# PacificBiosciences/portello

Hardware: AMD Instinct MI355X
Metric: lifted HiFi reads/sec (whole node) (higher is better)
Workload: dtype int32; 1 GPU; wgs30x; reads_total=2000000, reads_this_rank=2000000, read_len_mean=15000, items_per_gpu=2065417, in_ops_per_gpu=62827345, out_ops_per_gpu=56590310, large_items_per_gpu=0, mid_items_per_gpu=0, retry_items_per_gpu=0, lane_items_per_gpu=2065417, heavy_lane_items_per_gpu=0, seq_fmt=bam4, parallelism=one read set, 20 Mb windows dealt to 1 ranks by input ops, gather=none, launched_by=single process

## Files before the change

include/portello_liftover.h:

```cpp
#ifndef PORTELLO_LIFTOVER_H
#define PORTELLO_LIFTOVER_H

#include <stddef.h>
#include <stdint.h>

#ifdef __cplusplus
extern "C" {
#endif

#define PLO_API_VERSION 20

typedef enum plo_status {
    PLO_OK = 0,
    PLO_ERR_INVALID_ARG = 1,
    PLO_ERR_NO_DEVICE = 2,
    PLO_ERR_HIP = 3,
    PLO_ERR_OUT_OF_MEMORY = 4,
    PLO_ERR_RANGE = 5,
    PLO_ERR_INTERNAL = 6,
    PLO_ERR_IO = 7,
    PLO_ERR_DATA = 8
} plo_status;

enum {
    PLO_ITEM_LIFTED = 0,
    PLO_ITEM_NO_LIFTOVER = 1,
    PLO_ITEM_LEN_MISMATCH = 2,
    PLO_ITEM_PANIC = 3,
    PLO_ITEM_NEED_BASES = 4
};

enum {
    PLO_SEQ_BAM4 = 0,
// ... 92 lines not shown
    uint32_t n_big_items;
    uint64_t n_in_ops;
    uint64_t n_out_ops;
    uint64_t algo_bytes;
    float lanes_ms;
    float retry_ms;
    uint32_t n_lane_items;
    uint32_t n_retry_items;
    float mid_ms;
    uint32_t n_mid_items;
    uint32_t n_miss_items;
    float miss_ms;
    uint32_t tile_cap;
    uint32_t tile_window;
    float heavy_lanes_ms;
    uint32_t n_heavy_lane_items;
    float lane_utilisation;
    uint32_t heavy_kernel;
    uint32_t host_syncs;
} plo_timing;

plo_status plo_index_create(const plo_index_desc *desc, int device, plo_index **out);
void plo_index_destroy(plo_index *index);
plo_status plo_index_segment_map(const plo_index *index, uint32_t global_seg, uint32_t cap, int64_t *keys,
                                 int64_t *vals, uint32_t *n_entries);

plo_status plo_ctx_create(const plo_index *index, void *hip_stream, plo_ctx **out);
void plo_ctx_destroy(plo_ctx *ctx);
plo_status plo_ctx_set_stats(plo_ctx *ctx, int on);
plo_status plo_ctx_set_phase_events(plo_ctx *ctx, int on);

plo_status plo_liftover_batch(plo_ctx *ctx, const plo_batch_in *in, uint32_t stages, plo_batch_out *out);
plo_status plo_liftover_batch_dev(plo_ctx *ctx, const plo_batch_in *in, uint32_t stages, plo_batch_out *out);

typedef struct plo_finish_in {
    const uint16_t *read_flags;
    const uint8_t *qual;
    const uint64_t *read_qual_off;
    uint64_t qual_bytes;
} plo_finish_in;

#define PLO_NO_FLIP UINT64_MAX

typedef struct plo_finish_out {
    const uint16_t *item_flag;
    const uint16_t *item_bin;
// ... 509 lines not shown
```

portello_amd/abi.py:

```python
from __future__ import annotations

import ctypes as C
from dataclasses import dataclass, field
from typing import List, Optional, Sequence

import numpy as np

PLO_OK = 0
PLO_ERR_INVALID_ARG = 1
PLO_ERR_NO_DEVICE = 2
PLO_ERR_HIP = 3
PLO_ERR_OUT_OF_MEMORY = 4
PLO_ERR_RANGE = 5
PLO_ERR_INTERNAL = 6
PLO_ERR_IO = 7
PLO_ERR_DATA = 8

ITEM_LIFTED = 0
ITEM_NO_LIFTOVER = 1
ITEM_LEN_MISMATCH = 2
ITEM_PANIC = 3
ITEM_NEED_BASES = 4

SEQ_BAM4 = 0
# ... 85 lines not shown
        ("item_cseg", _u32p),
        ("seq_full", _u8p),
        ("read_seq_full_off", _u64p),
    ]


class PloBatchOut(C.Structure):
    _fields_ = [
        ("n_items", C.c_uint32),
        ("item_seg", _u32p),
        ("item_cseg", _u32p),
        ("item_status", _u8p),
        ("item_need_flipped", _u8p),
        ("item_mapq", _u8p),
        ("item_chrom_index", _u32p),
        ("item_ref_pos", _i64p),
        ("item_cigar_off", _u64p),
        ("item_cigar_len", _u32p),
        ("cigar", _u32p),
        ("n_cigar", C.c_uint64),
    ]


PLO_API_VERSION = 20


class PloTiming(C.Structure):
    _fields_ = [
        ("struct_size", C.c_uint32),
        ("total_ms", C.c_float),
        ("enumerate_ms", C.c_float),
        ("lift_ms", C.c_float),
        ("big_ms", C.c_float),
        ("n_items", C.c_uint32),
        ("n_big_items", C.c_uint32),
        ("n_in_ops", C.c_uint64),
        ("n_out_ops", C.c_uint64),
        ("algo_bytes", C.c_uint64),
        ("lanes_ms", C.c_float),
        ("retry_ms", C.c_float),
        ("n_lane_items", C.c_uint32),
        ("n_retry_items", C.c_uint32),
        ("mid_ms", C.c_float),
        ("n_mid_items", C.c_uint32),
        ("n_miss_items", C.c_uint32),
        ("miss_ms", C.c_float),
        ("tile_cap", C.c_uint32),
# ... 516 lines not shown
```

portello_amd/api.py:

```python
from __future__ import annotations

import ctypes as C
import os
from typing import Callable, List, Optional, Sequence, Tuple

import numpy as np

from . import abi
from . import cigar as cg

_HERE = os.path.dirname(os.path.abspath(__file__))
LIB_PATH = os.environ.get("PLO_LIB") or os.path.join(_HERE, "libportello_liftover.so")

Backend = Callable[[abi.IndexData, abi.BatchData, int], abi.BatchResult]


class PortelloError(RuntimeError):
    def __init__(self, status: int, msg: str):
        super().__init__(f"portello_liftover status {status}: {msg}")
        self.status = status


_lib = None


def load_library(path: Optional[str] = None):
    global _lib
    if _lib is not None and path is None:
        return _lib
    path = path or LIB_PATH
    if not os.path.exists(path):
        raise PortelloError(abi.PLO_ERR_NO_DEVICE, f"{path} not built: run `python -m portello_amd.build` (hipcc, gfx950)")
    try:
        import torch
    except ImportError:
        pass
    L = C.CDLL(path)
    vp = C.c_void_p
    if not hasattr(L, "plo_api_version") or L.plo_api_version() != abi.PLO_API_VERSION:
        raise PortelloError(abi.PLO_ERR_INVALID_ARG, f"{path} was built for another PLO_API_VERSION than this binding ({abi.PLO_API_VERSION}): rebuild it")
    L.plo_index_create.restype = C.c_int
    L.plo_index_create.argtypes = [C.POINTER(abi.PloIndexDesc), C.c_int, C.POINTER(vp)]
    L.plo_index_destroy.restype = None
    L.plo_index_destroy.argtypes = [vp]
    L.plo_index_segment_map.restype = C.c_int
    L.plo_index_segment_map.argtypes = [vp, C.c_uint32, C.c_uint32, C.POINTER(C.c_int64), C.POINTER(C.c_int64), C.POINTER(C.c_uint32)]
    L.plo_ctx_create.restype = C.c_int
    L.plo_ctx_create.argtypes = [vp, vp, C.POINTER(vp)]
    L.plo_ctx_destroy.restype = None
    L.plo_ctx_destroy.argtypes = [vp]
    L.plo_liftover_batch.restype = C.c_int
    L.plo_liftover_batch.argtypes = [vp, C.POINTER(abi.PloBatchIn), C.c_uint32, C.POINTER(abi.PloBatchOut)]
    L.plo_liftover_batch_dev.restype = C.c_int
    L.plo_liftover_batch_dev.argtypes = [vp, C.POINTER(abi.PloBatchIn), C.c_uint32, C.POINTER(abi.PloBatchOut)]
    L.plo_compact_output_dev.restype = C.c_int
    L.plo_compact_output_dev.argtypes = [vp, C.POINTER(abi.PloBatchOut)]
    L.plo_host_alloc.restype = C.c_int
    L.plo_host_alloc.argtypes = [C.c_size_t, C.POINTER(C.c_void_p)]
    L.plo_host_free.restype = None
    L.plo_host_free.argtypes = [C.c_void_p]
    L.plo_sa_segments_dev.restype = C.c_int
    L.plo_sa_segments_dev.argtypes = [vp, C.POINTER(abi.PloSaIn), C.POINTER(abi.PloSaOut)]
    L.plo_finish_batch_dev.restype = C.c_int
    L.plo_finish_batch_dev.argtypes = [vp, C.POINTER(abi.PloBatchIn), C.POINTER(abi.PloFinishIn), C.POINTER(abi.PloFinishOut)]
    L.plo_nm_dev.restype = C.c_int
    L.plo_nm_dev.argtypes = [vp, C.POINTER(abi.PloBatchIn), C.POINTER(abi.PloNmOut)]
    L.plo_md_dev.restype = C.c_int
# ... 93 lines not shown

    def __init__(self, data: abi.IndexData, device: int = 0):
        self.lib = load_library()
        self.data = data
        self._desc = data.to_desc()
        h = C.c_void_p()
        st = self.lib.plo_index_create(C.byref(self._desc), device, C.byref(h))
        if st != abi.PLO_OK:
            raise PortelloError(st, "plo_index_create failed" + (" (no usable HIP device)" if st == abi.PLO_ERR_NO_DEVICE else ""))
        self.handle = h
        self.device = device

    def segment_map(self, global_seg: int) -> Tuple[np.ndarray, np.ndarray]:
        n = C.c_uint32(0)
        self.lib.plo_index_segment_map(self.handle, global_seg, 0, None, None, C.byref(n))
        keys = np.zeros(max(1, n.value), dtype=np.int64)
        vals = np.zeros(max(1, n.value), dtype=np.int64)
        st = self.lib.plo_index_segment_map(self.handle, global_seg, n.value, keys.ctypes.data_as(C.POINTER(C.c_int64)),
                                            vals.ctypes.data_as(C.POINTER(C.c_int64)), C.byref(n))
        if st != abi.PLO_OK:
            raise PortelloError(st, "plo_index_segment_map")
        return keys[: n.value], vals[: n.value]

    def close(self):
        if getattr(self, "handle", None):
            self.lib.plo_index_destroy(self.handle)
            self.handle = None

    def __del__(self):
        try:
            self.close()
        except Exception:
            pass


class Engine:

    def __init__(self, index: Index, stream: Optional[int] = None):
        self.lib = index.lib
        self.index = index
        h = C.c_void_p()
        st = self.lib.plo_ctx_create(index.handle, C.c_void_p(stream) if stream else None, C.byref(h))
        if st != abi.PLO_OK:
            raise PortelloError(st, "plo_ctx_create failed")
        self.handle = h

# ... 373 lines not shown
```

portello_amd/build.py:

```python
from __future__ import annotations

import os
import subprocess
import sys

HERE = os.path.dirname(os.path.abspath(__file__))
CSRC = os.path.join(HERE, "csrc")
LIB = os.path.join(HERE, "libportello_liftover.so")
SOURCES = ["engine.hip", "bam_host.cpp", "phase1.cpp", "gather_rccl.cpp"]
LIBS = ["-lz", "-ldl"]
HEADERS = ["plo_wave.hpp", "lift_core.hpp", "lane_core.hpp", "lane_stream.hpp", "inflate.hpp", "deflate.hpp", "finish_core.hpp", "records_core.hpp", "batch_core.hpp", "aln_walk.hpp", "nm_core.hpp", "md_core.hpp", "eqx_core.hpp", "sort_core.hpp", "merge_core.hpp", "index_core.hpp", "depth_core.hpp", "pileup_core.hpp", "fasta_core.hpp", "window_core.hpp", "bgzf_walk.hpp", "lift_types.hpp", "index_pack.hpp", "enumerate.hpp", "bam_internal.hpp"]


def hipcc() -> str:
    for cand in (os.environ.get("HIPCC"), "/opt/rocm/bin/hipcc", "hipcc"):
        if cand and (os.path.isabs(cand) and os.path.exists(cand) or not os.path.isabs(cand)):
            return cand
    return "hipcc"


def source_hash() -> str:
    import hashlib

    h = hashlib.sha256()
    for f in sorted(["engine.hip"] + [x for x in HEADERS if x != "bam_internal.hpp"]):
        with open(os.path.join(CSRC, f), "rb") as fh:
            h.update(f.encode() + b"\0" + fh.read())
    return h.hexdigest()[:16]


def build_timing() -> str:
    out = os.path.join(HERE, "libportello_liftover_timing.so")
    cmd = [hipcc(), "--offload-arch=gfx950", "-O3", "-std=c++17", "-fPIC", "-shared", "-DPLO_PHASE_TIMING", "-I" + CSRC, "-o", out,
           os.path.join(CSRC, "engine.hip"), os.path.join(CSRC, "bam_host.cpp"), os.path.join(CSRC, "phase1.cpp"), os.path.join(CSRC, "gather_rccl.cpp")] + LIBS
# ... 21 lines not shown
```

portello_amd/csrc/engine.hip:

```cpp
#include <hip/hip_runtime.h>

#include <plo_wave.hpp>
#include <stdio.h>
#include <string.h>

#include <algorithm>
#include <atomic>
#include <chrono>
#include <map>
#include <mutex>
#include <string>
#include <vector>

#include "enumerate.hpp"
#include "finish_core.hpp"
#include "records_core.hpp"
#include "batch_core.hpp"
#include "nm_core.hpp"
#include "md_core.hpp"
#include "eqx_core.hpp"
#include "sort_core.hpp"
#include "merge_core.hpp"
#include "index_core.hpp"
#include "depth_core.hpp"
// ... 117 lines not shown
    if (bad) n = 0;
    seg_reflen[s] = (int)part;
    seg_readlen[s] = rpart > 0xfffffffeull ? 0xffffffffu : (uint32_t)rpart;
    seg_nm[s] = (c1 - c0) - pairs;
    seg_cnt[s] = n;
}

__global__ void k_item_emit(DevIndex ix, DevBatch bt, DevWork wk, uint32_t stages, const uint32_t *seg_off, int *seg_reflen, uint32_t item_cap, uint32_t *err) {
    uint32_t s = blockIdx.x * blockDim.x + threadIdx.x;
    if (s >= bt.n_segs) return;
    const uint32_t o0 = seg_off[s], o1 = seg_off[s + 1];
    if (o1 > item_cap) {
        if (o1 > o0) atomicOr(err, (uint32_t)VERR_CAP);
        return;
    }
    const int ref_len = seg_reflen[s];
    SegInfo si;
    seg_info_level0(si, bt, wk, stages, s);
    if (o0 == o1) return;
    seg_info_level1(si, ix, bt, wk, stages, s);
    bool neg = false;
    emit_segment_items(ix, wk, stages, s, o0, (long long)ref_len, si, &neg);
    if (neg) atomicOr(err, (uint32_t)VERR_RANGE);
}

__global__ __launch_bounds__(64) void k_map_build(const uint32_t *seg_cigar, const uint32_t *seg_cigar_off, const int64_t *seg_pos, uint32_t n_segments,
                                                  const uint32_t *kv_off, KV *kv, int *counts) {
    for (uint32_t g = blockIdx.x; g < n_segments; g += gridDim.x) {
        const uint32_t c0 = seg_cigar_off[g], c1 = seg_cigar_off[g + 1];
        const int cnt = build_segment_map_wave(seg_cigar + c0, c1 - c0, (long long)seg_pos[g], kv ? kv + kv_off[g] : nullptr);
        if (counts && threadIdx.x == 0) counts[g] = cnt;
    }
}

__global__ void k_item_desc(DevIndex ix, DevBatch bt, DevWork wk, uint32_t stages, const uint32_t *in_seg, const uint32_t *in_cseg,
                            uint32_t *err) {
    uint32_t i = blockIdx.x * blockDim.x + threadIdx.x;
    if (i >= wk.n_items) return;
    uint32_t seg = in_seg[i];
    {
        bool ok = seg < bt.n_segs;
        if (ok) {
            uint32_t contig = bt.seg_contig[seg];
            ok = contig < ix.n_contigs && in_cseg[i] < ix.contig_seg_off[contig + 1] - ix.contig_seg_off[contig];
        }
        if (!ok) {
// ... 1282 lines not shown

struct AlnPass {
    DevBuf len, off, partial;
    DevBuf out;
    DevBuf blk;
    HostBuf h;
    hipEvent_t ev[4] = {nullptr, nullptr, nullptr, nullptr};
    void release() {
        for (DevBuf *b : {&len, &off, &partial, &out, &blk}) b->release();
        h.release();
        for (hipEvent_t e : ev)
            if (e) (void)hipEventDestroy(e);
    }
};

}

struct plo_index {
    int device = 0;
    PackedIndex host;
    DevIndex d{};
    std::vector<void *> owned;
    uint32_t max_segs_per_contig = 0;
};

struct plo_fasta {
    int device = 0;
    hipStream_t stream = nullptr;
    hipEvent_t ev[6] = {nullptr, nullptr, nullptr, nullptr, nullptr, nullptr};
    bool emit_timed = false;
    bool byte_stores = false;
    std::string err;
    FaHost h;
    DevBuf text, tile_fn, tile_state, cnt, start, partial, blk, hdr, dest;
    HostBuf h_blk, h_hdr, h_dest;
    uint8_t *out = nullptr;
    size_t out_cap = 0;
    float ms = 0.f;
    bool finished = false;
    std::vector<int64_t> o_len;
    std::vector<const uint8_t *> o_ptr;
    std::vector<void *> adopted;
};

struct plo_depth {
    int device = 0;
// ... 355 lines not shown
            ix->owned.push_back(p);
            if (desc->chrom_len[c] > 0 && hipMemcpy(p, src, (size_t)desc->chrom_len[c], hipMemcpyHostToDevice) != hipSuccess)
                return fail(PLO_ERR_HIP);
            chrom_ptr[c] = (const uint8_t *)p;
        }
    }
    for (uint32_t c = 0; c < desc->n_contigs; ++c) {
        const uint8_t *src = desc->rev_contig_seq ? desc->rev_contig_seq[c] : nullptr;
        if (!src) continue;
        if (desc->seq_mem == PLO_MEM_DEVICE) {
            rev_ptr[c] = src;
        } else {
            void *p = nullptr;
            size_t bytes = std::max<size_t>((size_t)desc->contig_len[c], 16);
            if (hipMalloc(&p, bytes) != hipSuccess) return fail(PLO_ERR_OUT_OF_MEMORY);
            ix->owned.push_back(p);
            if (desc->contig_len[c] > 0 && hipMemcpy(p, src, (size_t)desc->contig_len[c], hipMemcpyHostToDevice) != hipSuccess)
                return fail(PLO_ERR_HIP);
            rev_ptr[c] = (const uint8_t *)p;
        }
    }
    if (upload(ix->owned, chrom_ptr, &d.chrom_seq) != hipSuccess) return fail(PLO_ERR_HIP);
    if (upload(ix->owned, rev_ptr, &d.contig_revseq) != hipSuccess) return fail(PLO_ERR_HIP);
    *out = ix;
    return PLO_OK;
}

void plo_index_destroy(plo_index *ix) {
    if (!ix) return;
    (void)hipSetDevice(ix->device);
    for (void *p : ix->owned) (void)hipFree(p);
    delete ix;
}

static thread_local std::string g_fasta_err;
#define FA_TRY(f, call)                                                                 \
    do {                                                                                \
        hipError_t _e = (call);                                                         \
        if (_e != hipSuccess) {                                                         \
            (f)->err = std::string(#call) + ": " + hipGetErrorString(_e);               \
            return (_e == hipErrorOutOfMemory) ? PLO_ERR_OUT_OF_MEMORY : PLO_ERR_HIP;   \
        }                                                                               \
    } while (0)

static void fasta_release(plo_fasta *f) {
    (void)hipSetDevice(f->device);
    if (f->stream) (void)hipStreamSynchronize(f->stream);
    for (DevBuf *b : {&f->text, &f->tile_fn, &f->tile_state, &f->cnt, &f->start, &f->partial, &f->blk, &f->hdr, &f->dest}) b->release();
    for (HostBuf *b : {&f->h_blk, &f->h_hdr, &f->h_dest}) b->release();
// ... 3529 lines not shown
```

portello_amd/csrc/lane_core.hpp:

```cpp
#pragma once
#include <plo_wave.hpp>
#include <stdint.h>

#include <type_traits>
#ifdef PLO_EMULATOR
#include <stdio.h>
#include <stdlib.h>
#endif

#include "lift_core.hpp"

#ifdef PLO_EMULATOR
#define PLO_MARK(s)
#else
#define PLO_MARK(s) asm volatile("; " s)
#endif

#ifndef PLO_SHIFT_LOCKSTEP
#define PLO_SHIFT_LOCKSTEP 1
#endif

namespace plo {



#ifdef PLO_EMULATOR
struct __attribute__((packed, aligned(4))) Ops4 {
    uint32_t x, y, z, w;
};
#else
typedef uint32_t Ops4 __attribute__((ext_vector_type(4), aligned(4)));
#endif
struct LaneOut {
// ... 127 lines not shown
            const bool keep = act & (t != OP_D);
            t = (t == OP_I) ? (int)OP_S : t;
            const bool same = keep & (run >= 16u) & (t == (int)(run & 15u));
            const bool flush = keep & !same & (run >= 16u);
            if (flush) o.R[w] = run;
            w += flush ? 1 : 0;
            const uint32_t add = (t == OP_P) ? 0u : ((uint32_t)L << 4);
            run = same ? run + add : (keep ? mk_op(t, L) : run);
        }
        {
            const bool flush = fix & (run >= 16u);
            if (flush) o.R[w] = run;
            w += flush ? 1 : 0;
            o.no = fix ? w : o.no;
        }
    }
}

struct XW16 {
    Ops4 r4, q4;
    uint32_t r1, q1;
    int rsh, qsh, jmin;
};
PLO_DEV bool xw16_issue(bool on, const uint8_t *ref, int ref_len, int r0, const ReadSeq &rd, int q0, const uint8_t *safe, XW16 &w, bool &miss) {
    bool ok = on & (r0 >= 0) & (q0 >= 0) & (q0 <= rd.len - 16);
    const int rsh = (int)(((unsigned)(uintptr_t)ref + (unsigned)r0) & 3u);
    ok = ok & (r0 - rsh >= 0) & (r0 - rsh <= ref_len - 20);
    const int jmin = rd.flip ? rd.len - q0 - 16 : q0;
    const bool bam4 = rd.fmt != PLO_SEQ_ASCII;
    int b0 = bam4 ? (jmin >> 1) : jmin;
    miss = false;
    if (rd.fmt == PLO_SEQ_BAM4_SPARSE) {
        const int j0 = ok ? jmin : 0, j1 = ok ? jmin + 15 : 0;
        const int g0 = j0 >> 5, g1 = j1 >> 5;
        const PLO_GLOBAL uint32_t *hdr = (const PLO_GLOBAL uint32_t *)(ok ? rd.p : safe);
        const uint32_t m0 = hdr[2 * (g0 >> 5)], rk0 = hdr[2 * (g0 >> 5) + 1], m1 = hdr[2 * (g1 >> 5)];
        const bool present = (((m0 >> (g0 & 31)) & (m1 >> (g1 & 31))) & 1u) != 0u;
        const unsigned rank = rk0 + (unsigned)__builtin_popcount(m0 & ((1u << (g0 & 31)) - 1u));
        const long long off = (long long)rd.data + (long long)rank * 16 + ((j0 >> 1) & 15);
        const bool bad = !present | (rank > 0x3ffffffu) | (off + (g1 - g0) * 16 + 20 > (long long)rd.hi);
        miss = ok & bad;
        ok = ok & !bad;
        b0 = (int)off;
    }
    const int qsh = (int)(((unsigned)(uintptr_t)rd.p + (unsigned)b0) & 3u);
    ok = ok & (b0 - qsh >= rd.lo) & (b0 - qsh + 20 <= rd.hi);
#ifdef PLO_EXP_PROBE_NOMEM
    const PLO_GLOBAL uint32_t *pr = (const PLO_GLOBAL uint32_t *)safe;
    const PLO_GLOBAL uint32_t *pq = (const PLO_GLOBAL uint32_t *)safe;
#else
    const PLO_GLOBAL uint32_t *pr = (const PLO_GLOBAL uint32_t *)(ok ? ref + (r0 - rsh) : safe);
    const PLO_GLOBAL uint32_t *pq = (const PLO_GLOBAL uint32_t *)(ok ? rd.p + (b0 - qsh) : safe);
#endif
    w.r4 = *(const PLO_GLOBAL Ops4 *)pr;
    w.r1 = pr[4];
    w.q4 = *(const PLO_GLOBAL Ops4 *)pq;
    w.q1 = pq[4];
    w.rsh = rsh;
    w.qsh = qsh;
    w.jmin = jmin;
    return ok;
}
PLO_DEV void xw16_decode(const ReadSeq &rd, const XW16 &wx, unsigned X[4]) {
    struct {
        unsigned wr[5], wq[5];
        int rsh, qsh, jmin;
    } w = {{wx.r4.x, wx.r4.y, wx.r4.z, wx.r4.w, wx.r1}, {wx.q4.x, wx.q4.y, wx.q4.z, wx.q4.w, wx.q1}, wx.rsh, wx.qsh, wx.jmin};
    const bool bam4 = rd.fmt != PLO_SEQ_ASCII;
    unsigned D[4];
    if (bam4) {
        unsigned S[5];
#pragma unroll
        for (int q = 0; q < 3; ++q) {
            unsigned Q = wv::align_bytes(w.wq[q + 1], w.wq[q], (unsigned)w.qsh);
            unsigned H = (Q >> 4) & 0x0f0f0f0fu, L = Q & 0x0f0f0f0fu;
            S[2 * q] = wv::perm_bytes(L, H, 0x05010400u);
            if (2 * q + 1 < 5) S[2 * q + 1] = wv::perm_bytes(L, H, 0x07030602u);
        }
        const unsigned par = (unsigned)(w.jmin & 1);
        const unsigned long long lo = rd.flip ? 0x4e4e4e434e47544eull : 0x565352474d43413dull;
        const unsigned long long hi = rd.flip ? 0x4e4e4e4e4e4e4e41ull : 0x4e42444b48595754ull;
#pragma unroll
        for (int v = 0; v < 4; ++v) {
            unsigned T = wv::align_bytes(S[v + 1], S[v], par);
            unsigned idx = T & 0x07070707u;
            unsigned dl = wv::perm_bytes((unsigned)(lo >> 32), (unsigned)lo, idx);
            unsigned dh = wv::perm_bytes((unsigned)(hi >> 32), (unsigned)hi, idx);
            unsigned mk = ((T >> 3) & 0x01010101u) * 0xffu;
            D[v] = (dh & mk) | (dl & ~mk);
        }
// ... 9 lines not shown
        unsigned R = wv::align_bytes(w.wr[u + 1], w.wr[u], (unsigned)w.rsh);
        unsigned B = rd.flip ? wv::perm_bytes(0u, D[3 - u], 0x00010203u) : D[u];
        X[u] = R ^ B;
    }
}

struct LaneProbe {
    XW16 w;
    int re = 0, qe = 0, maxk = 0;
    bool async_ok = false;
    bool miss = false;
};
PLO_DEV void lane_probe_arm(LaneProbe &p, bool on, int ref_len, int rs, int del, const ReadSeq &rd, int qs, int ins, int bound, bool &panic) {
    const int re = rs + del, qe = qs + ins;
    const int max_left = wv::imin(rs, qs);
    int maxk = wv::imin(max_left, bound);
    const bool bad = (max_left > 0) & ((re - 1 >= ref_len) | (qe - 1 >= rd.len));
    panic = panic | (on & bad);
    maxk = (bad | !on) ? 0 : maxk;
    p.re = re;
    p.qe = qe;
    p.maxk = maxk;
}
PLO_DEV void lane_probe_load(LaneProbe &p, bool on, const uint8_t *ref, int ref_len, const ReadSeq &rd, const uint8_t *safe) {
    p.async_ok = xw16_issue(on & (p.maxk > 0), ref, ref_len, p.re - 16, rd, p.qe - 16, safe, p.w, p.miss);
}
PLO_DEV int match_run_back_from(const uint8_t *ref, int ref_len, int re, ReadSeq &rd, int qe, int maxk, int k, int &probes) {
    while (k < maxk) {
        unsigned X[4];
        if (!xor_window16(ref, ref_len, re - k - 16, rd, qe - k - 16, X)) break;
        int n = wv::imin(16, maxk - k);
        int m = wv::imin(zero_bytes_from_top(X), n);
        probes += wv::imin(m + 1, n);
        k += m;
        if (m < n) return k;
    }
    while (k < maxk) {
        int n = wv::imin(8, maxk - k);
        int a[8], b[8];
#pragma unroll
        for (int j = 0; j < 8; ++j) {
            int jj = j < n ? j : 0;
            a[j] = ((const PLO_GLOBAL uint8_t *)ref)[re - 1 - k - jj];
            b[j] = read_base(rd, qe - 1 - k - jj);
        }
        int adv = n;
#pragma unroll
        for (int j = 7; j >= 0; --j)
            if (j < n && a[j] != b[j]) adv = j;
        probes += wv::imin(adv + 1, n);
        k += adv;
        if (adv < n) break;
    }
    return k;
}
PLO_DEV int top_zero_bytes(const unsigned X[4]) {
    const unsigned long long hi = ((unsigned long long)X[3] << 32) | X[2], lo = ((unsigned long long)X[1] << 32) | X[0];
    const int zh = hi ? (__builtin_clzll(hi) >> 3) : 8, zl = lo ? (__builtin_clzll(lo) >> 3) : 8;
    return hi ? zh : 8 + zl;
}
PLO_DEV int lane_probe_finish(const LaneProbe &p, bool on, const uint8_t *ref, int ref_len, ReadSeq &rd, int &probes) {
    unsigned X[4];
    xw16_decode(rd, p.w, X);
    const int n = wv::imin(16, p.maxk);
    const int m = wv::imin(top_zero_bytes(X), n);
    rd.miss = rd.miss | (on & p.miss);
    const bool live = on & (p.maxk > 0) & !p.miss;
    const bool fast = live & p.async_ok;
    int h = fast ? m : 0;
    probes += fast ? wv::imin(m + 1, n) : 0;
    const bool more = live & ((!p.async_ok) | ((m == n) & (n < p.maxk)));
    if (wv::ballot(more) != 0ull) {
        if (more) h = match_run_back_from(ref, ref_len, p.re, rd, p.qe, p.maxk, h, probes);
    }
    return h;
}

constexpr int LANE_RW = 20, LANE_WW = 28;
constexpr int LANE_WIN_DWORDS = LANE_RW + LANE_WW;
constexpr int LANE_WIN_MARGIN = 8;
constexpr int LANE_REGION_PAD = LANE_RW + 4;
struct LaneWin {
    uint32_t *G = nullptr;
    uint32_t *rw = nullptr, *ww = nullptr;
    int rbase = 0, wbase = 0;
};
PLO_DEV void win_fill(LaneWin &w, bool on, int idx) {
    if (on) {
        w.rbase = idx;
        Ops4 v[LANE_RW / 4];
#pragma unroll
        for (int q = 0; q < LANE_RW / 4; ++q) v[q] = *(const PLO_GLOBAL Ops4 *)(w.G + idx + 4 * q);
#pragma unroll
        for (int q = 0; q < LANE_RW / 4; ++q) {
            w.rw[(4 * q) * 64] = v[q].x;
            w.rw[(4 * q + 1) * 64] = v[q].y;
// ... 91 lines not shown
    if (has) {
        in_off = (int)wk.d.in_off[g];
        n_in = (int)wk.d.n_in[g];
        n_m = (int)wk.d.n_m[g];
        W0 = (int)wk.d.w0[g];
        W1 = (int)wk.d.w1[g];
        kv0 = (int)wk.d.kv0[g];
        kv1 = (int)wk.d.kv1[g];
        const uint32_t fl = wk.d.flags[g];
        pos1 = wk.d.pos1[g];
        seq_len = (int)wk.d.seq_len[g];
        const uint32_t read_len_in = wk.d.read_len[g];
        len_bad = read_len_in == 0xffffffffu || (uint32_t)seq_len != read_len_in;
        seq_off = wk.d.seq_off[g];
        shift_ref = wk.d.shift_ref[g];
        shift_ref_len = wk.d.shift_ref_len[g];
        rev = (fl & ITF_REV) != 0;
        flip = (fl & ITF_FLIP) != 0;
        const bool contig_fwd = (fl & ITF_CONTIG_FWD) != 0;
        do_shift = (stages & PLO_STAGE_LSHIFT) && (!(stages & PLO_STAGE_STRAND) || !contig_fwd);
    }
    const bool need_shift = do_shift;
    if constexpr (NOSHIFT) do_shift = false;
    const bool merges = do_shift || (stages & PLO_STAGE_LIFTOVER);
    const int n_ld = merges ? n_m : n_in;
    const int gap = has ? lane_region_gap(W0, W1) : 0;
    const int W = n_ld + gap + LANE_SLACK + (H16 ? H16_ALLOW : 0);
    const int W_dw = H16 ? (W + 1) >> 1 : W;

    int kvs_base = 0, kvs_cnt = 0;
    bool kv_lds = false, kvs_store = false;
    constexpr int KVS_Q = H16 ? LANE_KVS_MAX / 64 : LANE_KVS / 64;
    if constexpr (!H16) kvs_n = kvs_n < LANE_KVS ? kvs_n : LANE_KVS;
    KV kvs_e[KVS_Q];
#pragma unroll
    for (int q = 0; q < KVS_Q; ++q) kvs_e[q] = {0, 0};
    if (kvs != nullptr && (stages & PLO_STAGE_LIFTOVER)) {
        const int need_hi = wv::imin(kv1, W1 + 2);
        kvs_base = -wv::reduce_max(has ? -W0 : -IMAX);
        const int top = wv::reduce_max(has ? need_hi : 0);
        const int cnt = wv::imax(0, wv::imin(top - kvs_base, kvs_n));
        kv_lds = has & (need_hi <= kvs_base + cnt);
        kvs_cnt = cnt;
#pragma unroll
        for (int q = 0; q < KVS_Q; ++q)
            if (64 * q < kvs_n && lane + 64 * q < cnt) kvs_e[q] = ix.kv[kvs_base + lane + 64 * q];
// ... 256 lines not shown
                        const int t = op_type(c);
                        c_bad = c_bad | (have & (((unsigned)(t - (int)OP_S) >= 2u) | (c < 16u) | (t == pt)));
                        pt = have ? t : pt;
                        k += have ? 1 : 0;
                    }
                }
            }
            const bool lock_on = lk & !c_bad;
            if (wv::ballot(lock_on) != 0ull) {
                const uint8_t *const sref = (const uint8_t *)(uintptr_t)shift_ref;
                const int m0 = lock_on ? cur_off + n_lead : 0;
                int ref_head = pos1, read_head = lead_read, carry = 0, probes = 0;
                bool marked = false;
                LaneProbe pa, pb;
                int a_a = 0, a_b = 0;
                auto issue = [&](LaneProbe &p, int &a, int j) {
                    const bool on = lock_on & (j < ncl);
                    const uint32_t cm = R[on ? m0 + 2 * j : 0], cx = R[on ? m0 + 2 * j + 1 : 0];
                    const int t = op_type(cx), L = op_len(cx);
                    a = op_len(cm);
                    const int rs = ref_head + a, qs = read_head + a;
                    const int del = t == OP_D ? L : 0, ins = t == OP_I ? L : 0;
                    lane_probe_arm(p, on, shift_ref_len, rs, del, rd, qs, ins, IMAX, panic);
                    lane_probe_load(p, on, sref, shift_ref_len, rd, (const uint8_t *)plo_safe_words);
                    ref_head = on ? rs + del : ref_head;
                    read_head = on ? qs + ins : read_head;
                };
                auto resolve = [&](LaneProbe &p, int a, int j) {
                    const bool on = lock_on & (j < ncl);
                    const int bound = carry + a;
                    p.maxk = wv::imin(p.maxk, bound);
                    int h = lane_probe_finish(p, on, sref, shift_ref_len, rd, probes);
                    h = rd.miss ? 0 : h;
                    const int sh = wv::imin(bound, h);
                    if (on) R[m0 + 2 * j] = mk_op(OP_M, bound - sh);
                    marked = marked | (on & (bound == sh));
                    carry = on ? sh : carry;
                };
                PLO_MARK("LOCKSTEP LOOP BEGIN");
                issue(pa, a_a, 0);
                for (int j = 0; wv::ballot(lock_on & (j < ncl)) != 0ull; j += 2) {
                    PLO_LC(8, 2)
                    if constexpr (STATS) {
                        ctx.u_act += (unsigned)__builtin_popcountll(wv::ballot(lock_on & (j < ncl))) + (unsigned)__builtin_popcountll(wv::ballot(lock_on & (j + 1 < ncl)));
                        ctx.u_trips += 2;
                    }
                    issue(pb, a_b, j + 1);
                    resolve(pa, a_a, j);
                    issue(pa, a_a, j + 2);
                    resolve(pb, a_b, j + 1);
                }
                PLO_MARK("LOCKSTEP LOOP END");
                if (lock_on) R[m0 + 2 * ncl] = mk_op(OP_M, op_len(R[m0 + 2 * ncl]) + carry);
                if constexpr (STATS) algo += lock_on ? 2u * (unsigned)probes : 0u;
                const bool mk = lock_on & marked;
// ... 19 lines not shown
            }
        }
        if constexpr (!NOSHIFT) if (wv::ballot(shift_on) != 0ull) {
            const uint8_t *const sref = (const uint8_t *)(uintptr_t)shift_ref;
            LaneOut o;
            wr_open(o, gap);
            rd_fill(shift_on, cur_off);
            const int wl0 = cur_off - gap;
            const int wl_ext = W - gap;
            int k = 0;
            bool fin = !shift_on;
            int ref_head = pos1, read_head = 0, match = 0, del = 0, ins = 0, blk_ref = 0, blk_read = 0;
            bool in_blk = false, pend = false;
            int p_match = 0, p_ins = 0, p_del = 0, msince = 0, probes = 0;
            LaneProbe pr;
            PLO_MARK("SHIFT LOOP BEGIN");
            for (unsigned long long bm; (bm = wv::ballot(!fin)) != 0ull;) {
                PLO_LC(8, 1)
                if constexpr (STATS) {
                    ctx.u_act += (unsigned)__builtin_popcountll(bm);
                    ctx.u_trips += 1;
                }
                wr_room(o, shift_on, gap);
                if (wv::ballot(pend) != 0ull) lane_probe_load(pr, pend, sref, shift_ref_len, rd, (const uint8_t *)plo_safe_words);
                bool stop = fin, ev_other = false, ev_end = false;
                int ev_t = 0, ev_L = 0;
                while (wv::ballot(!stop) != 0ull) {
                    PLO_LC(9, 1)
                    const bool act = !stop;
                    const bool have = k < n;
                    rd_need(k, have & shift_on, shift_on);
                    const uint32_t c = rd_at(k, have & (!WIN | shift_on));
                    const int t = op_type(c), L = op_len(c);
                    const bool indel = have & b_is_indel(t);
                    const bool ism = have & b_is_match(t);
                    const bool other = have & !indel & !ism;
                    const bool atend = !have;
                    const bool ev = act & ((in_blk & (ism | other | atend)) | other | atend);
                    const bool take = act & !ev;
                    const bool memb = take & indel & (L > 0);
                    const bool open = memb & !in_blk;
                    blk_ref = open ? ref_head : blk_ref;
                    blk_read = open ? read_head : blk_read;
                    in_blk = in_blk | memb;
                    del += (memb & (t == OP_D)) ? L : 0;
                    ins += (memb & (t == OP_I)) ? L : 0;
                    const bool tm = take & ism;
                    msince += (tm & pend) ? L : 0;
                    match += (tm & !pend) ? L : 0;
                    read_head += (take & b_read_cons(t)) ? L : 0;
                    ref_head += (take & b_ref_cons(t)) ? L : 0;
                    k += take ? 1 : 0;
                    ev_t = ev ? t : ev_t;
                    ev_L = ev ? L : ev_L;
                    ev_other = ev ? other : ev_other;
                    ev_end = ev ? atend : ev_end;
                    stop = stop | ev;
                }
                const bool evl = !fin;
                const bool endc = evl & in_blk;
                const bool flushing = evl & (ev_other | ev_end);
                const int wl = ext ? wl_ext : wl0 + k;
                auto resolve = [&](bool on) {
                    int h = lane_probe_finish(pr, on, sref, shift_ref_len, rd, probes);
                    h = rd.miss ? 0 : h;
                    const int sh = wv::imin(p_match, h);
                    lane_push<false, ST, H16>(o, on & (p_match - sh > 0), OP_M, p_match - sh, wl);
                    lane_push<false, ST, H16>(o, on & (p_ins > 0), OP_I, p_ins, wl);
                    lane_push<false, ST, H16>(o, on & (p_del > 0), OP_D, p_del, wl);
                    match = on ? sh + msince : match;
                    msince = on ? 0 : msince;
                    pend = pend & !on;
                };
#pragma nounroll
                for (int pass = 0; pass < 2; ++pass) {
                    const bool res = (pass == 0 ? evl : flushing) & pend;
                    if (wv::ballot(res) != 0ull) {
                        if (pass == 1) lane_probe_load(pr, res, sref, shift_ref_len, rd, (const uint8_t *)plo_safe_words);
                        resolve(res);
                    }
                    if (pass == 1) break;
                    if (wv::ballot(endc) != 0ull) {
                        lane_probe_arm(pr, endc, shift_ref_len, blk_ref, del, rd, blk_read, ins, match, panic);
                        p_match = endc ? match : p_match;
                        p_ins = endc ? ins : p_ins;
                        p_del = endc ? del : p_del;
                        ins = endc ? 0 : ins;
                        del = endc ? 0 : del;
                        in_blk = in_blk & !endc;
                        pend = pend | endc;
                    }
                    if (wv::ballot(flushing & pend) == 0ull) break;
                }
                if (wv::ballot(flushing) != 0ull) {
                    lane_push<false, ST, H16>(o, flushing & (match > 0), OP_M, match, wl);
                    match = flushing ? 0 : match;
                    const bool oth = flushing & ev_other;
                    lane_push<true, ST, H16>(o, oth, ev_t, ev_L, wl + 1);
                    read_head += (oth & b_read_cons(ev_t)) ? ev_L : 0;
                    ref_head += (oth & b_ref_cons(ev_t)) ? ev_L : 0;
                    k += oth ? 1 : 0;
// ... 469 lines not shown
```

portello_amd/csrc/lift_types.hpp:

```cpp
#pragma once
#include <stdint.h>

#include "../../include/portello_liftover.h"

namespace plo {

enum : int { OP_M = 0, OP_I = 1, OP_D = 2, OP_N = 3, OP_S = 4, OP_H = 5, OP_P = 6, OP_EQ = 7, OP_X = 8 };
constexpr int NONE32 = (int)0x80000000;
constexpr int IMAX = 0x7fffffff;
constexpr int ITEM_NEED_BIG = 0xFF;
constexpr int MAXI = 64;
constexpr uint32_t sparse_header_bytes(uint32_t seq_len) { return ((((seq_len + 1023u) >> 10) * 8u) + 15u) & ~15u; }

struct alignas(8) KV {
    int key;
    int val;
};

struct DevIndex {
    const KV *kv;
    const uint32_t *cs_kv_off;
    const uint32_t *cs_chrom;
    const uint8_t *cs_is_fwd;
    const uint8_t *cs_mapq;
    const int *cs_start;
    const int *cs_end;
    const uint32_t *contig_seg_off;
    const int *contig_len;
    const uint8_t *const *contig_revseq;
    const uint8_t *const *chrom_seq;
    const int *chrom_len;
    uint32_t n_contigs, n_segments, n_chroms;
};

struct DevBatch {
    const uint8_t *read_is_reverse;
    const uint32_t *read_seq_len;
    const uint64_t *read_seq_off;
    const uint8_t *seq;
    int seq_fmt;
    uint64_t seq_bytes;
    const uint32_t *seg_read;
    const uint32_t *seg_contig;
    const int64_t *seg_pos;
    const uint8_t *seg_is_fwd;
    const uint32_t *seg_cigar_off;
    const uint32_t *cigar;
    uint32_t n_reads, n_segs;
};

enum { CNT_CIGAR = 0, CNT_OVERFLOW = 1, CNT_NBIG = 2, CNT_ALGO_BYTES = 3, CNT_IN_OPS = 4, CNT_ERROR = 5, CNT_OUT_OPS = 6, CNT_NRETRY = 7, CNT_PHASE0 = 8, CNT_NHUGE = 20, CNT_NMISS = 21, CNT_LANE_ACT = 22, CNT_LANE_TRIPS = 23, CNT_N = 24 };

struct ItemDesc {
    uint32_t *in_off;
    uint32_t *n_in;
// ... 62 lines not shown
```

Baseline: 1.605 billion reads/s.

## Pack contig reverse sequences to 4-bit form for faster shift-probe matching

```diff
diff --git a/include/portello_liftover.h b/include/portello_liftover.h
--- a/include/portello_liftover.h
+++ b/include/portello_liftover.h
@@ -8,7 +8,7 @@
 extern "C" {
 #endif
 
-#define PLO_API_VERSION 20
+#define PLO_API_VERSION 21
 
 typedef enum plo_status {
     PLO_OK = 0,
@@ -147,6 +147,7 @@
 
 plo_status plo_index_create(const plo_index_desc *desc, int device, plo_index **out);
 void plo_index_destroy(plo_index *index);
+uint32_t plo_index_packed_contigs(const plo_index *index);
 plo_status plo_index_segment_map(const plo_index *index, uint32_t global_seg, uint32_t cap, int64_t *keys,
                                  int64_t *vals, uint32_t *n_entries);
 
diff --git a/portello_amd/abi.py b/portello_amd/abi.py
--- a/portello_amd/abi.py
+++ b/portello_amd/abi.py
@@ -131,7 +131,7 @@
     ]
 
 
-PLO_API_VERSION = 20
+PLO_API_VERSION = 21
 
 
 class PloTiming(C.Structure):
diff --git a/portello_amd/api.py b/portello_amd/api.py
--- a/portello_amd/api.py
+++ b/portello_amd/api.py
@@ -43,6 +43,8 @@
     L.plo_index_create.argtypes = [C.POINTER(abi.PloIndexDesc), C.c_int, C.POINTER(vp)]
     L.plo_index_destroy.restype = None
     L.plo_index_destroy.argtypes = [vp]
+    L.plo_index_packed_contigs.restype = C.c_uint32
+    L.plo_index_packed_contigs.argtypes = [vp]
     L.plo_index_segment_map.restype = C.c_int
     L.plo_index_segment_map.argtypes = [vp, C.c_uint32, C.c_uint32, C.POINTER(C.c_int64), C.POINTER(C.c_int64), C.POINTER(C.c_uint32)]
     L.plo_ctx_create.restype = C.c_int
@@ -182,6 +184,9 @@
             raise PortelloError(st, "plo_index_segment_map")
         return keys[: n.value], vals[: n.value]
 
+    def packed_contigs(self) -> int:
+        return int(self.lib.plo_index_packed_contigs(self.handle))
+
     def close(self):
         if getattr(self, "handle", None):
             self.lib.plo_index_destroy(self.handle)
diff --git a/portello_amd/build.py b/portello_amd/build.py
--- a/portello_amd/build.py
+++ b/portello_amd/build.py
@@ -9,7 +9,7 @@
 LIB = os.path.join(HERE, "libportello_liftover.so")
 SOURCES = ["engine.hip", "bam_host.cpp", "phase1.cpp", "gather_rccl.cpp"]
 LIBS = ["-lz", "-ldl"]
-HEADERS = ["plo_wave.hpp", "lift_core.hpp", "lane_core.hpp", "lane_stream.hpp", "inflate.hpp", "deflate.hpp", "finish_core.hpp", "records_core.hpp", "batch_core.hpp", "aln_walk.hpp", "nm_core.hpp", "md_core.hpp", "eqx_core.hpp", "sort_core.hpp", "merge_core.hpp", "index_core.hpp", "depth_core.hpp", "pileup_core.hpp", "fasta_core.hpp", "window_core.hpp", "bgzf_walk.hpp", "lift_types.hpp", "index_pack.hpp", "enumerate.hpp", "bam_internal.hpp"]
+HEADERS = ["plo_wave.hpp", "lift_core.hpp", "lane_core.hpp", "seq_pack.hpp", "lane_stream.hpp", "inflate.hpp", "deflate.hpp", "finish_core.hpp", "records_core.hpp", "batch_core.hpp", "aln_walk.hpp", "nm_core.hpp", "md_core.hpp", "eqx_core.hpp", "sort_core.hpp", "merge_core.hpp", "index_core.hpp", "depth_core.hpp", "pileup_core.hpp", "fasta_core.hpp", "window_core.hpp", "bgzf_walk.hpp", "lift_types.hpp", "index_pack.hpp", "enumerate.hpp", "bam_internal.hpp"]
 
 
 def hipcc() -> str:
diff --git a/portello_amd/csrc/engine.hip b/portello_amd/csrc/engine.hip
--- a/portello_amd/csrc/engine.hip
+++ b/portello_amd/csrc/engine.hip
@@ -163,6 +163,14 @@
     bool neg = false;
     emit_segment_items(ix, wk, stages, s, o0, (long long)ref_len, si, &neg);
     if (neg) atomicOr(err, (uint32_t)VERR_RANGE);
+}
+
+__global__ __launch_bounds__(256) void k_seq4_pack(const uint8_t *src, int len, uint8_t *dst, int *bad) {
+    const long long nbytes = ((long long)len + 1) >> 1;
+    bool ok = true;
+    for (long long b = ((long long)blockIdx.x * blockDim.x + threadIdx.x) * 16; b < nbytes; b += (long long)gridDim.x * blockDim.x * 16)
+        ok = ok & seq4_pack_range(src, len, dst, b, b + 16 < nbytes ? b + 16 : nbytes);
+    if (!ok) atomicOr(bad, 1);
 }
 
 __global__ __launch_bounds__(64) void k_map_build(const uint32_t *seg_cigar, const uint32_t *seg_cigar_off, const int64_t *seg_pos, uint32_t n_segments,
@@ -1491,6 +1499,7 @@
     DevIndex d{};
     std::vector<void *> owned;
     uint32_t max_segs_per_contig = 0;
+    uint32_t n_packed = 0;
 };
 
 struct plo_fasta {
@@ -1892,9 +1901,41 @@
     }
     if (upload(ix->owned, chrom_ptr, &d.chrom_seq) != hipSuccess) return fail(PLO_ERR_HIP);
     if (upload(ix->owned, rev_ptr, &d.contig_revseq) != hipSuccess) return fail(PLO_ERR_HIP);
+    bool packed_on = true;
+    if (const char *e = getenv("PLO_SHIFT_PACKED")) packed_on = atoi(e) != 0;
+    if (packed_on) {
+        std::vector<const uint8_t *> rev4_ptr(desc->n_contigs, nullptr);
+        int *d_bad = nullptr;
+        if (hipMalloc((void **)&d_bad, 16) != hipSuccess) return fail(PLO_ERR_OUT_OF_MEMORY);
+        ix->owned.push_back(d_bad);
+        for (uint32_t c = 0; c < desc->n_contigs; ++c) {
+            const int len = desc->contig_len[c];
+            if (!rev_ptr[c] || len <= 0) continue;
+            const size_t bytes = seq4_alloc_bytes(len);
+            void *p = nullptr;
+            if (hipMalloc(&p, bytes) != hipSuccess) return fail(PLO_ERR_OUT_OF_MEMORY);
+            ix->owned.push_back(p);
+            if (hipMemset(p, 0, bytes) != hipSuccess || hipMemset(d_bad, 0, 4) != hipSuccess) return fail(PLO_ERR_HIP);
+            const long long chunks = ((((long long)len + 1) >> 1) + 15) / 16;
+            const uint32_t blocks = (uint32_t)std::min<long long>((chunks + 255) / 256, 65535ll * 4);
+            hipLaunchKernelGGL(k_seq4_pack, dim3(blocks), dim3(256), 0, 0, rev_ptr[c], len, (uint8_t *)p + SEQ4_FRONT, d_bad);
+            int bad = 0;
+            if (hipMemcpy(&bad, d_bad, 4, hipMemcpyDeviceToHost) != hipSuccess) return fail(PLO_ERR_HIP);
+            if (bad) {
+                ix->owned.pop_back();
+                (void)hipFree(p);
+                continue;
+            }
+            rev4_ptr[c] = (const uint8_t *)p + SEQ4_FRONT;
+            ++ix->n_packed;
+        }
+        if (ix->n_packed && upload(ix->owned, rev4_ptr, &d.contig_revseq4) != hipSuccess) return fail(PLO_ERR_HIP);
+    }
     *out = ix;
     return PLO_OK;
 }
+
+uint32_t plo_index_packed_contigs(const plo_index *ix) { return ix ? ix->n_packed : 0u; }
 
 void plo_index_destroy(plo_index *ix) {
     if (!ix) return;
diff --git a/portello_amd/csrc/lane_core.hpp b/portello_amd/csrc/lane_core.hpp
--- a/portello_amd/csrc/lane_core.hpp
+++ b/portello_amd/csrc/lane_core.hpp
@@ -9,6 +9,7 @@
 #endif
 
 #include "lift_core.hpp"
+#include "seq_pack.hpp"
 
 #ifdef PLO_EMULATOR
 #define PLO_MARK(s)
@@ -182,13 +183,18 @@
     uint32_t r1, q1;
     int rsh, qsh, jmin;
 };
-PLO_DEV bool xw16_issue(bool on, const uint8_t *ref, int ref_len, int r0, const ReadSeq &rd, int q0, const uint8_t *safe, XW16 &w, bool &miss) {
-    bool ok = on & (r0 >= 0) & (q0 >= 0) & (q0 <= rd.len - 16);
-    const int rsh = (int)(((unsigned)(uintptr_t)ref + (unsigned)r0) & 3u);
-    ok = ok & (r0 - rsh >= 0) & (r0 - rsh <= ref_len - 20);
+template <bool P4 = false>
+PLO_DEV bool xw16_issue(bool on, const uint8_t *ref, int ref_len, int r0, const ReadSeq &rd, int q0, const uint8_t *safe, XW16 &w, bool &miss, bool p4 = false) {
+    if constexpr (!P4) p4 = false;
+    bool ok = on & (q0 >= 0) & (q0 <= rd.len - 16);
+    const int rb = p4 ? seq4_window_byte(r0) : r0;
+    const int rsh = (int)(((unsigned)(uintptr_t)ref + (unsigned)rb) & 3u);
+    const bool r_ok = p4 ? ((unsigned)(r0 + 16) <= (unsigned)ref_len) : ((r0 >= 0) & (r0 - rsh >= 0) & (r0 - rsh <= ref_len - 20));
+    ok = ok & r_ok;
     const int jmin = rd.flip ? rd.len - q0 - 16 : q0;
     const bool bam4 = rd.fmt != PLO_SEQ_ASCII;
     int b0 = bam4 ? (jmin >> 1) : jmin;
+    b0 = p4 ? seq4_window_byte(jmin) : b0;
     miss = false;
     if (rd.fmt == PLO_SEQ_BAM4_SPARSE) {
         const int j0 = ok ? jmin : 0, j1 = ok ? jmin + 15 : 0;
@@ -209,23 +215,28 @@
     const PLO_GLOBAL uint32_t *pr = (const PLO_GLOBAL uint32_t *)safe;
     const PLO_GLOBAL uint32_t *pq = (const PLO_GLOBAL uint32_t *)safe;
 #else
-    const PLO_GLOBAL uint32_t *pr = (const PLO_GLOBAL uint32_t *)(ok ? ref + (r0 - rsh) : safe);
+    const PLO_GLOBAL uint32_t *pr = (const PLO_GLOBAL uint32_t *)(ok ? ref + (rb - rsh) : safe);
     const PLO_GLOBAL uint32_t *pq = (const PLO_GLOBAL uint32_t *)(ok ? rd.p + (b0 - qsh) : safe);
 #endif
     w.r4 = *(const PLO_GLOBAL Ops4 *)pr;
     w.r1 = pr[4];
     w.q4 = *(const PLO_GLOBAL Ops4 *)pq;
     w.q1 = pq[4];
-    w.rsh = rsh;
+    w.rsh = P4 ? (rsh | ((r0 & 1) << 2)) : rsh;
     w.qsh = qsh;
     w.jmin = jmin;
     return ok;
+}
+PLO_DEV int xw16_match4(const ReadSeq &rd, const XW16 &wx) {
+    const unsigned long long c = seq4_window(wx.r4.x, wx.r4.y, wx.r4.z, wx.r4.w, (unsigned)wx.rsh & 3u, (unsigned)wx.rsh >> 2);
+    const unsigned long long q = seq4_window(wx.q4.x, wx.q4.y, wx.q4.z, wx.q4.w, (unsigned)wx.qsh, (unsigned)wx.jmin & 1u);
+    return seq4_match_back(c, seq4_read_window(q, rd.flip != 0));
 }
 PLO_DEV void xw16_decode(const ReadSeq &rd, const XW16 &wx, unsigned X[4]) {
     struct {
         unsigned wr[5], wq[5];
         int rsh, qsh, jmin;
-    } w = {{wx.r4.x, wx.r4.y, wx.r4.z, wx.r4.w, wx.r1}, {wx.q4.x, wx.q4.y, wx.q4.z, wx.q4.w, wx.q1}, wx.rsh, wx.qsh, wx.jmin};
+    } w = {{wx.r4.x, wx.r4.y, wx.r4.z, wx.r4.w, wx.r1}, {wx.q4.x, wx.q4.y, wx.q4.z, wx.q4.w, wx.q1}, wx.rsh & 3, wx.qsh, wx.jmin};
     const bool bam4 = rd.fmt != PLO_SEQ_ASCII;
     unsigned D[4];
     if (bam4) {
@@ -281,9 +292,15 @@
     p.qe = qe;
     p.maxk = maxk;
 }
-PLO_DEV void lane_probe_load(LaneProbe &p, bool on, const uint8_t *ref, int ref_len, const ReadSeq &rd, const uint8_t *safe) {
-    p.async_ok = xw16_issue(on & (p.maxk > 0), ref, ref_len, p.re - 16, rd, p.qe - 16, safe, p.w, p.miss);
-}
+template <bool P4 = false>
+PLO_DEV void lane_probe_load(LaneProbe &p, bool on, const uint8_t *ref, int ref_len, const ReadSeq &rd, const uint8_t *safe, bool p4 = false) {
+    p.async_ok = xw16_issue<P4>(on & (p.maxk > 0), ref, ref_len, p.re - 16, rd, p.qe - 16, safe, p.w, p.miss, p4);
+}
+struct LaneAscii {
+    const uint8_t *const *revseq = nullptr;
+    const uint32_t *contig = nullptr;
+    uint32_t g = 0;
+};
 PLO_DEV int match_run_back_from(const uint8_t *ref, int ref_len, int re, ReadSeq &rd, int qe, int maxk, int k, int &probes) {
     while (k < maxk) {
         unsigned X[4];
@@ -318,11 +335,21 @@
     const int zh = hi ? (__builtin_clzll(hi) >> 3) : 8, zl = lo ? (__builtin_clzll(lo) >> 3) : 8;
     return hi ? zh : 8 + zl;
 }
-PLO_DEV int lane_probe_finish(const LaneProbe &p, bool on, const uint8_t *ref, int ref_len, ReadSeq &rd, int &probes) {
-    unsigned X[4];
-    xw16_decode(rd, p.w, X);
+template <bool P4 = false>
+PLO_DEV int lane_probe_finish(const LaneProbe &p, bool on, const uint8_t *ref, int ref_len, ReadSeq &rd, int &probes, bool p4 = false, const LaneAscii &asc = LaneAscii()) {
+    if constexpr (!P4) p4 = false;
+    int tz = 0;
+    if constexpr (P4) {
+        if (wv::ballot(on & p4) != 0ull) tz = xw16_match4(rd, p.w);
+    }
+    if (!P4 || wv::ballot(on & !p4) != 0ull) {
+        unsigned X[4];
+        xw16_decode(rd, p.w, X);
+        const int tb = top_zero_bytes(X);
+        tz = p4 ? tz : tb;
+    }
     const int n = wv::imin(16, p.maxk);
-    const int m = wv::imin(top_zero_bytes(X), n);
+    const int m = wv::imin(tz, n);
     rd.miss = rd.miss | (on & p.miss);
     const bool live = on & (p.maxk > 0) & !p.miss;
     const bool fast = live & p.async_ok;
@@ -330,7 +357,13 @@
     probes += fast ? wv::imin(m + 1, n) : 0;
     const bool more = live & ((!p.async_ok) | ((m == n) & (n < p.maxk)));
     if (wv::ballot(more) != 0ull) {
-        if (more) h = match_run_back_from(ref, ref_len, p.re, rd, p.qe, p.maxk, h, probes);
+        if (more) {
+            const uint8_t *aref = ref;
+            if constexpr (P4) {
+                if (p4) aref = asc.revseq[asc.contig[asc.g]];
+            }
+            h = match_run_back_from(aref, ref_len, p.re, rd, p.qe, p.maxk, h, probes);
+        }
     }
     return h;
 }
@@ -468,6 +501,22 @@
     }
     const bool need_shift = do_shift;
     if constexpr (NOSHIFT) do_shift = false;
+    constexpr bool P4 = !WIN && !H16 && !SP && !NOSHIFT;
+    bool p4 = false;
+    LaneAscii asc;
+    (void)p4;
+    (void)asc;
+    if constexpr (P4) {
+        if (ix.contig_revseq4 != nullptr && bt.seq_fmt == PLO_SEQ_BAM4) {
+            const uint32_t cg = (has & do_shift) ? wk.d.contig[g] : 0u;
+            const unsigned long long r4 = (unsigned long long)(uintptr_t)ix.contig_revseq4[cg];
+            p4 = has & do_shift & (r4 != 0ull);
+            shift_ref = p4 ? r4 : shift_ref;
+            asc.revseq = ix.contig_revseq;
+            asc.contig = wk.d.contig;
+            asc.g = g;
+        }
+    }
     const bool merges = do_shift || (stages & PLO_STAGE_LIFTOVER);
     const int n_ld = merges ? n_m : n_in;
     const int gap = has ? lane_region_gap(W0, W1) : 0;
@@ -770,7 +819,7 @@
                     const int rs = ref_head + a, qs = read_head + a;
                     const int del = t == OP_D ? L : 0, ins = t == OP_I ? L : 0;
                     lane_probe_arm(p, on, shift_ref_len, rs, del, rd, qs, ins, IMAX, panic);
-                    lane_probe_load(p, on, sref, shift_ref_len, rd, (const uint8_t *)plo_safe_words);
+                    lane_probe_load<P4>(p, on, sref, shift_ref_len, rd, (const uint8_t *)plo_safe_words, p4);
                     ref_head = on ? rs + del : ref_head;
                     read_head = on ? qs + ins : read_head;
                 };
@@ -778,7 +827,7 @@
                     const bool on = lock_on & (j < ncl);
                     const int bound = carry + a;
                     p.maxk = wv::imin(p.maxk, bound);
-                    int h = lane_probe_finish(p, on, sref, shift_ref_len, rd, probes);
+                    int h = lane_probe_finish<P4>(p, on, sref, shift_ref_len, rd, probes, p4, asc);
                     h = rd.miss ? 0 : h;
                     const int sh = wv::imin(bound, h);
                     if (on) R[m0 + 2 * j] = mk_op(OP_M, bound - sh);
@@ -844,7 +893,7 @@
                     ctx.u_trips += 1;
                 }
                 wr_room(o, shift_on, gap);
-                if (wv::ballot(pend) != 0ull) lane_probe_load(pr, pend, sref, shift_ref_len, rd, (const uint8_t *)plo_safe_words);
+                if (wv::ballot(pend) != 0ull) lane_probe_load<P4>(pr, pend, sref, shift_ref_len, rd, (const uint8_t *)plo_safe_words, p4);
                 bool stop = fin, ev_other = false, ev_end = false;
                 int ev_t = 0, ev_L = 0;
                 while (wv::ballot(!stop) != 0ull) {
@@ -884,7 +933,7 @@
                 const bool flushing = evl & (ev_other | ev_end);
                 const int wl = ext ? wl_ext : wl0 + k;
                 auto resolve = [&](bool on) {
-                    int h = lane_probe_finish(pr, on, sref, shift_ref_len, rd, probes);
+                    int h = lane_probe_finish<P4>(pr, on, sref, shift_ref_len, rd, probes, p4, asc);
                     h = rd.miss ? 0 : h;
                     const int sh = wv::imin(p_match, h);
                     lane_push<false, ST, H16>(o, on & (p_match - sh > 0), OP_M, p_match - sh, wl);
@@ -898,7 +947,7 @@
                 for (int pass = 0; pass < 2; ++pass) {
                     const bool res = (pass == 0 ? evl : flushing) & pend;
                     if (wv::ballot(res) != 0ull) {
-                        if (pass == 1) lane_probe_load(pr, res, sref, shift_ref_len, rd, (const uint8_t *)plo_safe_words);
+                        if (pass == 1) lane_probe_load<P4>(pr, res, sref, shift_ref_len, rd, (const uint8_t *)plo_safe_words, p4);
                         resolve(res);
                     }
                     if (pass == 1) break;
diff --git a/portello_amd/csrc/lift_types.hpp b/portello_amd/csrc/lift_types.hpp
--- a/portello_amd/csrc/lift_types.hpp
+++ b/portello_amd/csrc/lift_types.hpp
@@ -31,6 +31,7 @@
     const uint8_t *const *chrom_seq;
     const int *chrom_len;
     uint32_t n_contigs, n_segments, n_chroms;
+    const uint8_t *const *contig_revseq4 = nullptr;
 };
 
 struct DevBatch {
diff --git a/portello_amd/csrc/seq_pack.hpp b/portello_amd/csrc/seq_pack.hpp
--- /dev/null
+++ b/portello_amd/csrc/seq_pack.hpp
@@ -0,0 +1,71 @@
+#pragma once
+#include <plo_wave.hpp>
+#include <stddef.h>
+#include <stdint.h>
+
+namespace plo {
+
+constexpr int SEQ4_FRONT = 16;
+constexpr int SEQ4_BACK = 24;
+PLO_HD size_t seq4_alloc_bytes(int len) { return ((size_t)SEQ4_FRONT + (size_t)((len + 1) >> 1) + (size_t)SEQ4_BACK + 15u) & ~(size_t)15; }
+
+PLO_HD int seq4_code(unsigned c) {
+    const unsigned long long lo = 0x00f30c00b400d2e1ull, hi = 0x0000000a09708650ull;
+    const unsigned i = c - (unsigned)'A';
+    const bool letter = i < 25u && ((0x016e34cfu >> i) & 1u) != 0u;
+    const int code = (int)(((i < 16u ? lo : hi) >> (4u * (i & 15u))) & 15u);
+    return letter ? code : (c == (unsigned)'=' ? 0 : -1);
+}
+PLO_HD bool seq4_pack_range(const uint8_t *src, int len, uint8_t *dst, long long byte_begin, long long byte_end) {
+    bool ok = true;
+    for (long long b = byte_begin; b < byte_end; ++b) {
+        const long long i = 2 * b;
+        const int h = i < (long long)len ? seq4_code(src[i]) : 0, l = i + 1 < (long long)len ? seq4_code(src[i + 1]) : 0;
+        ok = ok & (h >= 0) & (l >= 0);
+        dst[b] = (uint8_t)(((h & 15) << 4) | (l & 15));
+    }
+    return ok;
+}
+
+PLO_DEV unsigned seq4_alignbit(unsigned hi, unsigned lo, unsigned sh) {
+#ifdef PLO_EMULATOR
+    return (unsigned)(((((unsigned long long)hi) << 32) | lo) >> (sh & 31u));
+#else
+    return __builtin_amdgcn_alignbit(hi, lo, sh);
+#endif
+}
+PLO_DEV unsigned seq4_brev32(unsigned w) {
+#ifdef PLO_EMULATOR
+    w = ((w >> 1) & 0x55555555u) | ((w & 0x55555555u) << 1);
+    w = ((w >> 2) & 0x33333333u) | ((w & 0x33333333u) << 2);
+    w = ((w >> 4) & 0x0f0f0f0fu) | ((w & 0x0f0f0f0fu) << 4);
+    return (w >> 24) | ((w >> 8) & 0xff00u) | ((w << 8) & 0xff0000u) | (w << 24);
+#else
+    return __builtin_bitreverse32(w);
+#endif
+}
+PLO_DEV int seq4_window_byte(int pos) { return (pos >> 1) - 1; }
+PLO_DEV unsigned long long seq4_window(unsigned w0, unsigned w1, unsigned w2, unsigned w3, unsigned bsh, unsigned par) {
+    const unsigned sel = wv::perm_bytes(0u, bsh & 3u, 0u) + 0x00010203u;
+    const unsigned b0 = wv::perm_bytes(w1, w0, sel), b1 = wv::perm_bytes(w2, w1, sel), b2 = wv::perm_bytes(w3, w2, sel);
+    const unsigned sh = 24u - 4u * (par & 1u);
+    return (((unsigned long long)seq4_alignbit(b0, b1, sh)) << 32) | seq4_alignbit(b1, b2, sh);
+}
+PLO_DEV unsigned seq4_flip32(unsigned w) {
+    w = seq4_brev32(w);
+    const unsigned s1 = w >> 1, t1 = w & s1, o1 = w | s1;
+    const unsigned multi = (t1 | (t1 >> 2)) | (o1 & (o1 >> 2));
+    const unsigned none = ~(o1 | (o1 >> 2));
+    const unsigned bad = (multi | none) & 0x11111111u;
+    return w | ((bad << 4) - bad);
+}
+PLO_DEV unsigned long long seq4_read_window(unsigned long long stored, bool flip) {
+    const unsigned long long f = (((unsigned long long)seq4_flip32((unsigned)stored)) << 32) | seq4_flip32((unsigned)(stored >> 32));
+    return flip ? f : stored;
+}
+PLO_DEV int seq4_match_back(unsigned long long contig, unsigned long long read) {
+    const unsigned long long x = contig ^ read;
+    return x ? (__builtin_ctzll(x) >> 2) : 16;
+}
+
+}
```

Measured after the change: 1.604 billion reads/s. About the same (-0.1%).
